# caiyuanhao1998/Open-DiffusionGS

Hardware: AMD Instinct MI355X
Metric: novel-view renders/sec (DiT step + GS raster) at 256^2 (higher is better)
Workload: dtype bf16; 1 GPU; obj-256 sampling step (BASELINE.json configs[2]): DGSDenoiser.forward = DiT image_to_gaussians (width 1024, 24 blocks, L=4098, bf16 MFMA, fp32 accumulate) + 4 fp32 rasterizations of P=262146 Gaussians at 256^2 per sample; random-init weights; batch_per_gpu=1, views=4, resolution=256, gaussians=262146, parallelism=dp1

## Files before the change

open-diffusiongs_amd/csrc/raster_forward.hip:

```cpp
#include <string.h>

#include "raster_cells.h"

namespace dgs {

struct FwdParams {
    int P, D, M, W, H, V, vps, gx, gy, T;
    const float *bg, *means3D, *shs, *colors_pre, *opac, *scales, *rots, *cov_pre, *viewm, *projm, *campos, *tanfov;
    float tanfovx, tanfovy, scale_mod;
    int prefiltered, raw_act;
    int bin_mode;
    int bitonic_cap;
    int bitonic_any;
    int exact_exp;
    int debug;
    int* radii;
    float* out_color;
    float *out_depth, *out_alpha;
    GeomState g;
    ImageState im;
    BinningState bn;
};

__device__ __forceinline__ void view_tanfov(const FwdParams& p, int v, float* tx, float* ty) {
    if (p.tanfov) { *tx = p.tanfov[2 * v]; *ty = p.tanfov[2 * v + 1]; }
    else { *tx = p.tanfovx; *ty = p.tanfovy; }
}

__device__ __forceinline__ void sh_to_rgb(int deg, const float* sh, float dx, float dy, float dz, float* out, unsigned* clamp_bits) {
    const float len = sqrtf(dx * dx + dy * dy + dz * dz);
    const float x = dx / len, y = dy / len, z = dz / len;
    unsigned bits = 0;
#pragma unroll
    for (int c = 0; c < 3; ++c) {
#define SH(k) sh[3 * (k) + c]
        float r = 0.28209479177387814f * SH(0);
        if (deg > 0) {
            r = r - 0.4886025119029199f * y * SH(1) + 0.4886025119029199f * z * SH(2) - 0.4886025119029199f * x * SH(3);
            if (deg > 1) {
                const float xx = x * x, yy = y * y, zz = z * z, xy = x * y, yz = y * z, xz = x * z;
                r = r + 1.0925484305920792f * xy * SH(4) + -1.0925484305920792f * yz * SH(5) +
                    0.31539156525252005f * (2.0f * zz - xx - yy) * SH(6) + -1.0925484305920792f * xz * SH(7) +
                    0.5462742152960396f * (xx - yy) * SH(8);
                if (deg > 2) {
                    r = r + -0.5900435899266435f * y * (3.0f * xx - yy) * SH(9) + 2.890611442640554f * xy * z * SH(10) +
                        -0.4570457994644658f * y * (4.0f * zz - xx - yy) * SH(11) +
                        0.3731763325901154f * z * (2.0f * zz - 3.0f * xx - 3.0f * yy) * SH(12) +
                        -0.4570457994644658f * x * (4.0f * zz - xx - yy) * SH(13) + 1.445305721320277f * z * (xx - yy) * SH(14) +
                        -0.5900435899266435f * x * (xx - 3.0f * yy) * SH(15);
                }
            }
        }
#undef SH
        r += 0.5f;
        if (r < 0) bits |= 1u << c;
        out[c] = fmaxf(r, 0.0f);
    }
    *clamp_bits = bits;
}

__device__ __forceinline__ bool preprocess_one(const FwdParams& p, int v, int idx, int* rx0, int* ry0, int* rx1, int* ry1, uint32_t* depth_key) {
    const int s = v / p.vps;
    const size_t gi = (size_t)v * p.P + idx;
    const size_t si = (size_t)s * p.P + idx;
    p.radii[gi] = 0;
    p.g.tiles_touched[gi] = 0;
    p.g.keys[0][gi] = 0xFFFFFFFFu;
    const float* vm = p.viewm + 16 * v;
    const float* pm = p.projm + 16 * v;
    const float mx = p.means3D[3 * si], my = p.means3D[3 * si + 1], mz = p.means3D[3 * si + 2];
    const float hx = pm[0] * mx + pm[4] * my + pm[8] * mz + pm[12];
    const float hy = pm[1] * mx + pm[5] * my + pm[9] * mz + pm[13];
    const float hw = pm[3] * mx + pm[7] * my + pm[11] * mz + pm[15];
    const float pw = 1.0f / (hw + 0.0000001f);
    const float projx = hx * pw, projy = hy * pw;
    float tx = vm[0] * mx + vm[4] * my + vm[8] * mz + vm[12];
    float ty = vm[1] * mx + vm[5] * my + vm[9] * mz + vm[13];
    const float tz = vm[2] * mx + vm[6] * my + vm[10] * mz + vm[14];
    if (tz <= 0.2f) {
        if (p.prefiltered) p.im.totals[1] = DGS_ERR_PREFILTERED_CULLED;
        return false;
    }
    float tanx, tany;
    view_tanfov(p, v, &tanx, &tany);
    const float focal_y = p.H / (2.0f * tany), focal_x = p.W / (2.0f * tanx);

    float c6[6];
    if (p.cov_pre) {
#pragma unroll
        for (int k = 0; k < 6; ++k) c6[k] = p.cov_pre[6 * si + k];
    } else {
        cov3d_from_scale_rot(p.scales + 3 * si, p.rots + 4 * si, p.raw_act != 0, p.scale_mod, c6);
        if (p.debug) {
#pragma unroll
            for (int k = 0; k < 6; ++k) p.g.cov3D[6 * gi + k] = c6[k];
        }
    }
    const float limx = 1.3f * tanx, limy = 1.3f * tany;
    const float txtz = tx / tz, tytz = ty / tz;
    tx = fminf(limx, fmaxf(-limx, txtz)) * tz;
    ty = fminf(limy, fmaxf(-limy, tytz)) * tz;
    const M3 J = m3_cols(focal_x / tz, 0.0f, -(focal_x * tx) / (tz * tz), 0.0f, focal_y / tz, -(focal_y * ty) / (tz * tz), 0, 0, 0);
    const M3 Wm = m3_cols(vm[0], vm[4], vm[8], vm[1], vm[5], vm[9], vm[2], vm[6], vm[10]);
    const M3 Tm = m3_mul(Wm, J);
    const M3 Vrk = m3_cols(c6[0], c6[1], c6[2], c6[1], c6[3], c6[4], c6[2], c6[4], c6[5]);
    const M3 cov = m3_mul(m3_mul(m3_t(Tm), m3_t(Vrk)), Tm);
    const float ca = cov.c[0][0] + 0.3f, cb = cov.c[0][1], cc = cov.c[1][1] + 0.3f;
    const float det = ca * cc - cb * cb;
    if (det == 0.0f) return false;
    const float det_inv = 1.f / det;
    const float conx = cc * det_inv, cony = -cb * det_inv, conz = ca * det_inv;
    const float mid = 0.5f * (ca + cc);
    const float l1 = mid + sqrtf(fmaxf(0.1f, mid * mid - det));
    const float l2 = mid - sqrtf(fmaxf(0.1f, mid * mid - det));
    const float my_radius = ceilf(3.f * sqrtf(fmaxf(l1, l2)));
    const float px = (float)(((projx + 1.0) * p.W - 1.0) * 0.5);
    const float py = (float)(((projy + 1.0) * p.H - 1.0) * 0.5);
    const int irad = f2i_sat(my_radius);
    int x0, y0, x1, y1;
    tile_rect(px, py, irad, p.gx, p.gy, &x0, &y0, &x1, &y1);
    if ((x1 - x0) * (y1 - y0) == 0) return false;
    float rgb[3];
    unsigned cbits = 0;
    if (p.colors_pre) {
        rgb[0] = p.colors_pre[3 * si]; rgb[1] = p.colors_pre[3 * si + 1]; rgb[2] = p.colors_pre[3 * si + 2];
    } else {
        const float* cam = p.campos + 3 * v;
        sh_to_rgb(p.D, p.shs + 3 * (size_t)p.M * si, mx - cam[0], my - cam[1], mz - cam[2], rgb, &cbits);
    }
    float op = p.opac[si];
    if (p.raw_act) op = 1.0f / (1.0f + det_expf(-op));
    const float cut = (op > 0.0f) ? (__logf(1.0f / (255.0f * op)) - 0.004f) : __builtin_inff();
    p.g.depths[gi] = tz;
    p.radii[gi] = irad;
    p.g.means2D[gi] = make_float2(px, py);
    BlendRecord* rec = p.g.blend + gi;
    rec->co = make_float4(conx, cony, conz, op);
    rec->rc = make_float4(rgb[0], rgb[1], rgb[2], cut);
    *reinterpret_cast<float4*>(&rec->xy) = make_float4(px, py, tz, 0.f);
    p.g.clamped[gi] = (uint8_t)cbits;
    p.g.tiles_touched[gi] = (uint32_t)((y1 - y0) * (x1 - x0));
    p.g.keys[0][gi] = __float_as_uint(tz);
    *depth_key = __float_as_uint(tz);
    *rx0 = x0; *ry0 = y0; *rx1 = x1; *ry1 = y1;
    return true;
}

template <bool LDS_HIST>
__global__ __launch_bounds__(256) void preprocess_kernel(FwdParams p) {
    DGS_DYNAMIC_LDS(smem);
    uint32_t* lhist = reinterpret_cast<uint32_t*>(smem);
    const int v = blockIdx.y;
    const int idx = blockIdx.x * 256 + threadIdx.x;
    if (LDS_HIST) {
        for (int i = threadIdx.x; i < p.T; i += 256) lhist[i] = 0;
        __syncthreads();
    }
    if (blockIdx.x == 0) {
        uint32_t* w = p.g.range_ws + (size_t)v * range_ws_stride(p.P);
        for (int i = threadIdx.x; i <= kRangeBuckets; i += 256) w[i] = 0u;
    }
    int x0 = 0, y0 = 0, x1 = 0, y1 = 0;
    bool vis = false;
    uint32_t depth_key = 0xFFFFFFFFu;
    if (idx < p.P) vis = preprocess_one(p, v, idx, &x0, &y0, &x1, &y1, &depth_key);
    {
        __shared__ uint32_t s_rng[2][4];
        const uint32_t key = vis ? depth_key : 0xFFFFFFFFu;
        uint32_t hi = key != 0xFFFFFFFFu ? key : 0u, lo_c = key != 0xFFFFFFFFu ? ~key : 0u;
#pragma unroll
        for (int o = 32; o > 0; o >>= 1) { hi = max(hi, (uint32_t)__shfl_xor((int)hi, o)); lo_c = max(lo_c, (uint32_t)__shfl_xor((int)lo_c, o)); }
        if ((threadIdx.x & 63) == 0) { s_rng[0][threadIdx.x >> 6] = hi; s_rng[1][threadIdx.x >> 6] = lo_c; }
        __syncthreads();
        if (threadIdx.x < 2) {
            const uint32_t m = max(max(s_rng[threadIdx.x][0], s_rng[threadIdx.x][1]), max(s_rng[threadIdx.x][2], s_rng[threadIdx.x][3]));
            if (m) atomicMax(p.im.depth_range + ((size_t)threadIdx.x * p.V + v) * kRangeSlots + (blockIdx.x % kRangeSlots), m);
        }
    }
    uint32_t* gcount = p.im.tile_count + (size_t)v * p.T;
    if (vis) {
        uint32_t* const grid = LDS_HIST ? lhist : gcount;
        atomicAdd(&grid[y0 * p.gx + x0], 1u);
        if (x1 < p.gx) atomicAdd(&grid[y0 * p.gx + x1], 0xffffffffu);
        if (y1 < p.gy) {
            atomicAdd(&grid[y1 * p.gx + x0], 0xffffffffu);
            if (x1 < p.gx) atomicAdd(&grid[y1 * p.gx + x1], 1u);
        }
    }
    if (LDS_HIST) {
        __syncthreads();
        for (int i = threadIdx.x; i < p.T; i += 256) {
            const uint32_t c = lhist[i];
            if (c) atomicAdd(&gcount[i], c);
        }
    }
}

__global__ __launch_bounds__(256) void radix_hist_kernel(const uint32_t* keys, uint32_t* hist, int P, int NB, int shift) {
    __shared__ uint32_t h[256];
    const int v = blockIdx.y, b = blockIdx.x;
    h[threadIdx.x] = 0;
    __syncthreads();
    const uint32_t* k = keys + (size_t)v * P;
    const int base = b * kSortTile;
#pragma unroll 4
    for (int r = 0; r < kSortItems; ++r) {
        const int i = base + r * 256 + threadIdx.x;
        if (i < P) atomicAdd(&h[(k[i] >> shift) & 255u], 1u);
    }
    __syncthreads();
    hist[((size_t)v * NB + b) * 256 + threadIdx.x] = h[threadIdx.x];
}

__global__ __launch_bounds__(256) void radix_colscan_kernel(uint32_t* hist, uint32_t* base, int NB) {
    __shared__ uint32_t scratch[8];
    const int v = blockIdx.y, d = threadIdx.x;
    uint32_t* h = hist + (size_t)v * NB * 256;
    uint32_t run = 0;
    for (int b0 = 0; b0 < NB; b0 += 16) {
        uint32_t c[16];
#pragma unroll
        for (int u = 0; u < 16; ++u) c[u] = (b0 + u < NB) ? h[(size_t)(b0 + u) * 256 + d] : 0u;
#pragma unroll
        for (int u = 0; u < 16; ++u) {
            if (b0 + u < NB) h[(size_t)(b0 + u) * 256 + d] = run;
            run += c[u];
        }
    }
    uint32_t total;
    const uint32_t ex = block_exclusive_scan<256>(run, scratch, &total);
    base[v * 256 + d] = ex;
}

__global__ __launch_bounds__(256) void radix_scatter_kernel(const uint32_t* keys_in, const uint32_t* vals_in, uint32_t* keys_out,
                                                           uint32_t* vals_out, uint32_t* rank_of, const uint32_t* hist,
                                                           const uint32_t* base, int P, int NB, int shift) {
    __shared__ uint32_t wcount[4][256];
    __shared__ uint32_t running[256];
    const int v = blockIdx.y, b = blockIdx.x, tid = threadIdx.x;
    const int lane = tid & 63, wave = tid >> 6;
    const size_t vo = (size_t)v * P;
    running[tid] = base[v * 256 + tid] + hist[((size_t)v * NB + b) * 256 + tid];
    const unsigned long long lt_mask = (lane == 0) ? 0ull : (~0ull >> (64 - lane));
    for (int r = 0; r < kSortItems; ++r) {
#pragma unroll
        for (int w = 0; w < 4; ++w) wcount[w][tid] = 0;
        __syncthreads();
        const int i = b * kSortTile + r * 256 + tid;
        const bool valid = i < P;
        const uint32_t key = valid ? keys_in[vo + i] : 0xFFFFFFFFu;
        const uint32_t val = valid ? (vals_in ? vals_in[vo + i] : (uint32_t)i) : 0u;
        const uint32_t dig = (key >> shift) & 255u;
        unsigned long long peers = __ballot(valid);
#pragma unroll
        for (int bit = 0; bit < 8; ++bit) {
            const unsigned long long m = __ballot((dig >> bit) & 1u);
            peers &= ((dig >> bit) & 1u) ? m : ~m;
        }
        const uint32_t rank_in_wave = (uint32_t)__popcll(peers & lt_mask);
        if (valid && rank_in_wave == 0) wcount[wave][dig] = (uint32_t)__popcll(peers);
        __syncthreads();
        if (valid) {
            uint32_t pos = running[dig] + rank_in_wave;
            for (int w = 0; w < wave; ++w) pos += wcount[w][dig];
            keys_out[vo + pos] = key;
            vals_out[vo + pos] = val;
            if (rank_of) rank_of[vo + val] = pos;
        }
        __syncthreads();
        running[tid] += wcount[0][tid] + wcount[1][tid] + wcount[2][tid] + wcount[3][tid];
    }
}

struct RangeMap {
    uint32_t lo; float scale; bool any;
    __device__ __forceinline__ uint32_t bucket(uint32_t key) const { return min((uint32_t)((float)(key - lo) * scale), (uint32_t)kRangeBuckets - 1u); }
};
__device__ __forceinline__ RangeMap range_map(const uint32_t* depth_range, int V, int v, uint32_t* s_map ) {
    if (threadIdx.x < 64) {
        const int which = threadIdx.x >> 5, slot = threadIdx.x & 31;
        uint32_t x = slot < kRangeSlots ? depth_range[((size_t)which * V + v) * kRangeSlots + slot] : 0u;
#pragma unroll
        for (int o = 16; o > 0; o >>= 1) x = max(x, (uint32_t)__shfl_xor((int)x, o));
        if (slot == 0) s_map[which] = x;
    }
    __syncthreads();
    const uint32_t hi_w = s_map[0], lo_w = s_map[1];
    const uint32_t hi = hi_w, lo = ~lo_w;
    RangeMap m;
    m.any = (hi_w | lo_w) != 0u;
    m.lo = m.any ? lo : 0u;
    m.scale = m.any ? (float)kRangeBuckets / ((float)(hi - lo) + 1.0f) : 0.f;
    return m;
}

__global__ __launch_bounds__(256) void range_count_kernel(const uint32_t* keys, const uint32_t* depth_range, uint32_t* ws, int P, int V, int stride) {
    __shared__ uint32_t h[kRangeBuckets];
    __shared__ uint32_t s_c[4];
    __shared__ uint32_t s_map[2];
    const int v = blockIdx.y, b = blockIdx.x, tid = threadIdx.x;
    const RangeMap m = range_map(depth_range, V, v, s_map);
    for (int i = tid; i < kRangeBuckets; i += 256) h[i] = 0;
    __syncthreads();
    const uint32_t* k = keys + (size_t)v * P;
    uint32_t culled = 0;
#pragma unroll 4
    for (int r = 0; r < kRangeItems; ++r) {
        const int i = b * kRangeTile + r * 256 + tid;
        if (i < P) {
            const uint32_t key = k[i];
            if (key != 0xFFFFFFFFu) atomicAdd(&h[m.bucket(key)], 1u); else ++culled;
        }
    }
#pragma unroll
    for (int o = 32; o > 0; o >>= 1) culled += (uint32_t)__shfl_xor((int)culled, o);
    if ((tid & 63) == 0) s_c[tid >> 6] = culled;
    __syncthreads();
    uint32_t* w = ws + (size_t)v * stride;
    for (int i = tid; i < kRangeBuckets; i += 256) { const uint32_t c = h[i]; if (c) atomicAdd(&w[i], c); }
    if (tid == 0) w[2 * kRangeBuckets + 1 + b] = (s_c[0] + s_c[1]) + (s_c[2] + s_c[3]);
}

__global__ __launch_bounds__(1024) void range_plan_kernel(uint32_t* ws, int NB, int NWIN, int stride) {
    __shared__ uint32_t scratch[20];
    __shared__ uint32_t s_start[kRangeBuckets + 1];
    uint32_t* w = ws + (size_t)blockIdx.x * stride;
    const int tid = threadIdx.x;
    const uint32_t c = tid < kRangeBuckets ? w[tid] : 0u;
    uint32_t nvis;
    const uint32_t ex = block_exclusive_scan<1024>(c, scratch, &nvis);
    __syncthreads();
    if (tid < kRangeBuckets) { w[tid] = ex; w[kRangeBuckets + 1 + tid] = 0u; s_start[tid] = ex; }
    if (tid == 0) { w[kRangeBuckets] = nvis; s_start[kRangeBuckets] = nvis; }
    __syncthreads();
    for (int j = tid; j <= NWIN; j += 1024) {
        const uint32_t want = (uint32_t)j * (uint32_t)kRangeWindow;
        int lo = 0, hi = kRangeBuckets;
        while (lo < hi) { const int mid = (lo + hi) >> 1; if (s_start[mid] < want) lo = mid + 1; else hi = mid; }
        w[2 * kRangeBuckets + 1 + NB + j] = j == NWIN ? nvis : s_start[lo];
    }
    const uint32_t cc = tid < NB ? w[2 * kRangeBuckets + 1 + tid] : 0u;
    uint32_t all;
    const uint32_t cex = block_exclusive_scan<1024>(cc, scratch, &all);
    if (tid < NB) w[2 * kRangeBuckets + 1 + tid] = nvis + cex;
}

__global__ __launch_bounds__(256) void range_scatter_kernel(const uint32_t* keys, const uint32_t* depth_range, uint32_t* ws, uint32_t* keys_out,
                                                           uint32_t* vals_out, uint32_t* order, uint32_t* rank_of, int P, int V, int stride) {
    __shared__ uint32_t h[kRangeBuckets];
    __shared__ uint32_t s_cc[kRangeItems][4];
    __shared__ uint32_t s_map[2];
    const int v = blockIdx.y, b = blockIdx.x, tid = threadIdx.x, lane = tid & 63, wave = tid >> 6;
    const RangeMap m = range_map(depth_range, V, v, s_map);
    const size_t vo = (size_t)v * P;
    uint32_t* w = ws + (size_t)v * stride;
    for (int i = tid; i < kRangeBuckets; i += 256) h[i] = 0;
    __syncthreads();
    uint32_t key[kRangeItems], slot[kRangeItems];
    const unsigned long long lt_mask = (lane == 0) ? 0ull : (~0ull >> (64 - lane));
#pragma unroll
    for (int r = 0; r < kRangeItems; ++r) {
        const int i = b * kRangeTile + r * 256 + tid;
        key[r] = i < P ? keys[vo + i] : 0u;
        const bool in = i < P, cul = in && key[r] == 0xFFFFFFFFu;
        slot[r] = (in && !cul) ? atomicAdd(&h[m.bucket(key[r])], 1u) : 0u;
        const unsigned long long cm = __ballot(cul);
        if (cul) slot[r] = (uint32_t)__popcll(cm & lt_mask);
        if (lane == 0) s_cc[r][wave] = (uint32_t)__popcll(cm);
    }
    __syncthreads();
    {
        constexpr int Q = kRangeBuckets / 256;
        uint32_t c[Q], st0[Q], got[Q];
#pragma unroll
        for (int q = 0; q < Q; ++q) { c[q] = h[tid + 256 * q]; st0[q] = w[tid + 256 * q]; }
#pragma unroll
        for (int q = 0; q < Q; ++q) got[q] = c[q] ? atomicAdd(&w[kRangeBuckets + 1 + tid + 256 * q], c[q]) : 0u;
#pragma unroll
        for (int q = 0; q < Q; ++q) h[tid + 256 * q] = st0[q] + got[q];
    }
    __syncthreads();
    const uint32_t cbase = w[2 * kRangeBuckets + 1 + b];
#pragma unroll
    for (int r = 0; r < kRangeItems; ++r) {
        const int i = b * kRangeTile + r * 256 + tid;
        if (i >= P) continue;
        if (key[r] != 0xFFFFFFFFu) {
            const uint32_t pos = h[m.bucket(key[r])] + slot[r];
            keys_out[vo + pos] = key[r];
            vals_out[vo + pos] = (uint32_t)i;
        } else {
            uint32_t off = 0;
            for (int q = 0; q < r; ++q) off += (s_cc[q][0] + s_cc[q][1]) + (s_cc[q][2] + s_cc[q][3]);
            for (int q = 0; q < wave; ++q) off += s_cc[r][q];
            const uint32_t pos = cbase + off + slot[r];
            order[vo + pos] = (uint32_t)i;
            rank_of[vo + i] = pos;
        }
    }
}

__global__ __launch_bounds__(1024) void scan_tiles_kernel(uint32_t* count, uint2* ranges, uint32_t* cursor, int n,
                                                         int32_t* totals, long long capacity, uint32_t* order, int gx, int gy,
                                                         int32_t* stats_dev, int32_t* stats_host) {
    __shared__ uint32_t scratch[20];
    __shared__ uint32_t smax;
    __shared__ uint32_t s_class[1024];
    {
        const int T = gx * gy, V = n / T;
        for (int r = threadIdx.x; r < V * gy; r += 1024) {
            uint32_t* row = count + (size_t)(r / gy) * T + (size_t)(r % gy) * gx;
            uint32_t run = 0;
            for (int x0 = 0; x0 < gx; x0 += 16) {
                uint32_t c[16];
#pragma unroll
                for (int u = 0; u < 16; ++u) c[u] = x0 + u < gx ? row[x0 + u] : 0u;
#pragma unroll
                for (int u = 0; u < 16; ++u)
                    if (x0 + u < gx) { run += c[u]; row[x0 + u] = run; }
            }
        }
        __syncthreads();
        for (int cidx = threadIdx.x; cidx < V * gx; cidx += 1024) {
            uint32_t* col = count + (size_t)(cidx / gx) * T + (cidx % gx);
            uint32_t run = 0;
            for (int y0 = 0; y0 < gy; y0 += 16) {
                uint32_t c[16];
#pragma unroll
                for (int u = 0; u < 16; ++u) c[u] = y0 + u < gy ? col[(size_t)(y0 + u) * gx] : 0u;
#pragma unroll
                for (int u = 0; u < 16; ++u)
                    if (y0 + u < gy) { run += c[u]; col[(size_t)(y0 + u) * gx] = run; }
            }
        }
        __syncthreads();
    }
    uint32_t carry = 0, mx = 0;
    if (threadIdx.x == 0) smax = 0;
    for (int base = 0; base < n; base += 1024) {
        const int i = base + threadIdx.x;
        const uint32_t c = (i < n) ? count[i] : 0u;
        mx = max(mx, c);
        uint32_t tot;
        const uint32_t ex = block_exclusive_scan<1024>(c, scratch, &tot);
        if (i < n) { ranges[i] = make_uint2(carry + ex, carry + ex + c); cursor[i] = 0; }
        carry += tot;
    }
    __syncthreads();
    atomicMax(&smax, mx);
    __syncthreads();
    if (threadIdx.x == 0) {
        totals[0] = (int32_t)carry;
        totals[2] = (int32_t)smax;
        if (capacity >= 0 && (long long)carry > capacity) totals[1] = DGS_ERR_BINNING_OVERFLOW;
        const int32_t st1 = totals[1];
        if (stats_dev) { stats_dev[0] = (int32_t)carry; stats_dev[1] = st1; stats_dev[2] = (int32_t)smax; stats_dev[3] = 1; }
        if (stats_host) {
            stats_host[0] = (int32_t)carry; stats_host[1] = st1; stats_host[2] = (int32_t)smax;
            __threadfence_system();
            *reinterpret_cast<volatile int32_t*>(stats_host + 3) = 1;
        }
    }
    deal_tiles(count, n, smax, order, s_class, scratch);
}

enum { kFormRankSort = 1, kFormScan = 2, kFormBitonic = 3 };
__host__ __device__ __forceinline__ int binning_form_of(int bin_mode, int bitonic_cap, long long num_rendered, long long longest,
                                                        long long T, long long P, long long V, bool any_len = false) {
    const bool fits = bitonic_cap > 0 && (any_len || longest <= bitonic_cap);
    if (bin_mode == kFormScan || bin_mode == kFormRankSort) return bin_mode;
    if (bin_mode == kFormBitonic) return fits ? kFormBitonic : kFormRankSort;
    if (num_rendered * 10 >= T * P * V) return kFormScan;
    return fits ? kFormBitonic : kFormRankSort;
}
__host__ __device__ __forceinline__ bool scan_form_possible(int gx, int gy, long long T, long long P) {
    return gx <= 255 && gy <= 255 && T * P <= (1ll << 31);
}
__device__ __forceinline__ int binning_form(const FwdParams& p) {
    return binning_form_of(p.bin_mode, p.bitonic_cap, (long long)(uint32_t)p.im.totals[0], (long long)(uint32_t)p.im.totals[2], p.T, p.P, p.V,
                           p.bitonic_any != 0);
}
__device__ __forceinline__ bool binning_is_scan(const FwdParams& p) { return binning_form(p) == kFormScan; }

template <bool LDS_AGG>
__global__ __launch_bounds__(256) void emit_instances_kernel(FwdParams p) {
    DGS_DYNAMIC_LDS(smem);
    uint32_t* lcnt = reinterpret_cast<uint32_t*>(smem);
    uint32_t* lbase = lcnt + p.T;
    const int form = binning_form(p);
    if (p.im.totals[1] != 0 || form == kFormScan) return;
    const bool wide = form == kFormBitonic;
    const int v = blockIdx.y;
    const int idx = blockIdx.x * 256 + threadIdx.x;
    const size_t gi = (size_t)v * p.P + idx;
    int x0 = 0, y0 = 0, x1 = 0, y1 = 0;
    bool vis = false;
    if (idx < p.P && p.radii[gi] > 0) {
// ... 423 lines not shown
            const unsigned long long m = __ballot(tx - x0 < x1 - x0) & __ballot(ty - y0 < y1 - y0);
            if (EMIT) {
                const bool set = (m >> lane) & 1ull;
                slot[u] = off + cnt + (uint32_t)__popcll(m & lanes_before);
                val[u] = set ? order[rank0 + 64u * u] : 0u;
                setm |= (uint32_t)set << u;
            }
            cnt += (uint32_t)__popcll(m);
        }
        if (EMIT) {
#pragma unroll
            for (int u = 0; u < 8; ++u)
                if (((setm >> u) & 1u) && list_at + slot[u] < list_cap) {
                    ring[(ring_at + slot[u]) & (kRing - 1u)] = val[u];
                    list[list_at + slot[u]] = val[u];
                }
        }
    }
    return cnt;
}

__device__ __forceinline__ void scan_more(const FwdParams& p, TileScan& s, uint32_t* ring, uint32_t* scratch, const uint32_t* rects,
                                          const uint32_t* order, uint32_t* list, uint32_t count, uint32_t tx, uint32_t ty, int lane, int wave,
                                          unsigned long long lanes_before) {
    const uint32_t P = (uint32_t)p.P;
    unsigned long long want = 768ull * P / (count ? count : 1u);
    uint32_t win = (uint32_t)(want > (1ull << 24) ? (1ull << 24) : want);
    win = max(1024u, (win + 255u) & ~255u);
    const uint32_t room = kRing - s.waiting;
    uint32_t total = 0, off = 0;
    int g0 = 0, g1 = 0;
    for (;;) {
        const int groups = (int)((min(win, P - s.next_rank) + 63u) / 64u);
        const int gpw = (groups + 3) / 4;
        g0 = wave * gpw; g1 = min(groups, g0 + gpw);
        const uint32_t cnt = scan_groups<false>(rects, order, s.next_rank, g0, g1, P, tx, ty, lane, lanes_before, 0u, nullptr, 0u, nullptr, 0u, 0u);
        if (lane == 0) scratch[wave] = cnt;
        __syncthreads();
        total = 0; off = 0;
#pragma unroll
        for (int w = 0; w < 4; ++w) {
            const uint32_t c = scratch[w];
            if (w < wave) off += c;
            total += c;
        }
        __syncthreads();
        if (total <= room || win <= 256u) break;
        win = max(256u, (win / 2u + 255u) & ~255u);
    }
    scan_groups<true>(rects, order, s.next_rank, g0, g1, P, tx, ty, lane, lanes_before, off, ring, s.head + s.waiting, list, s.found, count);
    __syncthreads();
    s.next_rank += min(win, P - s.next_rank);
    s.found += total;
    s.waiting += total;
}

template <bool SCAN, bool FAST_EXP, bool AUX = false>
__global__ __launch_bounds__(256) void blend_forward_kernel(FwdParams p) {
    __shared__ CellXY<AUX> s_xy[256];
    __shared__ float4 s_co[256];
    __shared__ float4 s_rgbc[256];
    __shared__ uint4 s_cnt[16];
    __shared__ uint8_t s_list[17][256];
    __shared__ uint32_t s_walk[4];
    __shared__ uint2 s_stat[kRasterStats ? 4 : 1];
    __shared__ uint32_t s_ring[SCAN ? kRing : 1];
    __shared__ uint32_t s_scan[4];
    if (binning_is_scan(p) != SCAN) return;
    const uint32_t vt = p.im.tile_order[blockIdx.x];
    const int v = (int)(vt / (uint32_t)p.T), tile = (int)(vt % (uint32_t)p.T);
    const int bx = tile % p.gx, by = tile / p.gx;
    const int tid = threadIdx.x, lane = tid & 63, row = lane >> 4;
    const int wave = __builtin_amdgcn_readfirstlane(tid >> 6);
    const int cell = wave * 4 + row;
    const int pxi = bx * kTile + 4 * row + (lane & 3), pyi = by * kTile + 4 * wave + ((lane >> 2) & 3);
    const bool inside = pxi < p.W && pyi < p.H;
    const float pfx = (float)pxi, pfy = (float)pyi;
    const float tx0 = (float)(bx * kTile), ty0 = (float)(by * kTile);
    const unsigned long long lanes_before = (lane == 0) ? 0ull : (~0ull >> (64 - lane));
    const bool ok = p.im.totals[1] == 0;
    uint2 rg = p.im.ranges[vt];
    if (!ok) rg.y = rg.x;
    const int rounds = (int)((rg.y - rg.x + 255u) / 256u);
    const size_t vo = (size_t)v * p.P;
    const uint32_t* rects = p.g.vals[1] + vo;
    const uint32_t* order = p.g.vals[0] + vo;
    TileScan ts{0u, 0u, 0u, 0u};
    bool done = !inside;
    float T = 1.0f, C0 = 0.f, C1 = 0.f, C2 = 0.f;
    float Dz = 0.f;
    uint32_t last_contributor = 0;
    uint32_t st_entries = 0, st_trips = 0, st_batches = 0;
    for (int i = 0; i < rounds; ++i) {
        if (__syncthreads_count(done) == 256) break;
        if constexpr (kRasterStats) ++st_batches;
        const uint32_t pos = rg.x + (uint32_t)i * 256u + (uint32_t)tid;
        const uint32_t need = min(256u, rg.y - rg.x - (uint32_t)i * 256u);
        if (SCAN) {
            while (ts.waiting < need && ts.next_rank < (uint32_t)p.P)
                scan_more(p, ts, s_ring, s_scan, rects, order, p.bn.point_list + rg.x, rg.y - rg.x, (uint32_t)bx, (uint32_t)by, lane, wave, lanes_before);
        }
        const bool has = pos < rg.y && (!SCAN || (uint32_t)tid < ts.waiting);
        uint32_t id = 0u;
        if (has) id = SCAN ? s_ring[(ts.head + (uint32_t)tid) & (kRing - 1u)] : p.bn.point_list[pos];
        const unsigned m16[1] = {stage_entry<AUX>(has, p.g.blend + vo, nullptr, id, tid, tx0, ty0, s_xy, s_co, s_rgbc)};
        const uint32_t kept = compact_cells<1>(m16, cell, tid, lane, wave, lanes_before, s_cnt, s_list);
        if (SCAN) { const uint32_t took = min(need, ts.waiting); ts.head += took; ts.waiting -= took; }
        const uint32_t base = (uint32_t)i * 256u;
        const unsigned long long alive = __ballot(!done);
        if (alive != 0ull) {
            const uint32_t tot = (((alive >> (16 * row)) & 0xFFFFull) != 0ull) ? kept : 0u;
            uint32_t tot_l = done ? 0u : tot;
            using Entry = CellEntry<AUX>;
            auto load = [&](uint32_t j) { return Entry{s_xy[j], s_co[j], s_rgbc[j]}; };
            auto step = [&](uint32_t k, uint32_t j, const Entry& e) {
                const float dx = e.xy.x - pfx, dy = e.xy.y - pfy;
                const float power = -0.5f * (e.co.x * dx * dx + e.co.z * dy * dy) - e.co.y * dx * dy;
                const bool pass = (k < tot_l) & !(power > 0.0f) & !(power < e.rc.w);
                if (wave_ballot(pass) != 0ull) {
                    const float alpha = alpha_clamp(e.co.w * blend_exp<FAST_EXP>(pass ? power : 0.0f, e.co.w));
                    const float test_T = T * (1 - alpha);
                    const bool contributes = pass & !(alpha < 1.0f / 255.0f);
                    const bool finishes = contributes & (test_T < 0.0001f);
                    const bool blends = contributes & !finishes;
                    tot_l = finishes ? 0u : tot_l;
                    if constexpr (FAST_EXP) {
                        const float w = blends ? alpha * T : 0.0f;
                        C0 = __builtin_fmaf(e.rc.x, w, C0); C1 = __builtin_fmaf(e.rc.y, w, C1); C2 = __builtin_fmaf(e.rc.z, w, C2);
                        if constexpr (AUX) Dz = __builtin_fmaf(e.xy.z, w, Dz);
                    } else {
                        const float c0 = C0 + e.rc.x * alpha * T, c1 = C1 + e.rc.y * alpha * T, c2 = C2 + e.rc.z * alpha * T;
                        C0 = blends ? c0 : C0;
                        C1 = blends ? c1 : C1;
                        C2 = blends ? c2 : C2;
                        if constexpr (AUX) { const float dz = Dz + e.xy.z * alpha * T; Dz = blends ? dz : Dz; }
                    }
                    T = blends ? test_T : T;
                    last_contributor = blends ? base + j + 1u : last_contributor;
                }
            };
            const uint32_t k = walk_cell(s_list[cell], load, step, [&](uint32_t at) { return wave_ballot(at < tot_l) != 0ull; });
            done = done | (tot_l != tot);
            if constexpr (kRasterStats) { st_entries += min(tot, k); st_trips += k; }
        }
    }
    if (inside) {
        const size_t pid = (size_t)p.W * pyi + pxi;
        const size_t HW = (size_t)p.H * p.W;
        p.im.final_T[(size_t)v * HW + pid] = T;
        p.im.n_contrib[(size_t)v * HW + pid] = last_contributor;
        float* out = p.out_color + (size_t)v * 3 * HW;
        const float bad = __uint_as_float(0x7FC00000u);
        out[pid] = ok ? C0 + T * p.bg[0] : bad;
        out[HW + pid] = ok ? C1 + T * p.bg[1] : bad;
        out[2 * HW + pid] = ok ? C2 + T * p.bg[2] : bad;
        if constexpr (AUX) {
            p.out_depth[(size_t)v * HW + pid] = ok ? Dz : bad;
            p.out_alpha[(size_t)v * HW + pid] = ok ? 1.0f - T : bad;
        }
    }
    uint32_t walked = last_contributor;
#pragma unroll
    for (int o = 32; o > 0; o >>= 1) walked = max(walked, (uint32_t)__shfl_xor((int)walked, o));
    uint2 stat = make_uint2(0u, 0u);
    if constexpr (kRasterStats) stat = tile_stat_sums<4>((lane & 15) == 0, st_entries, st_trips, lane, wave, s_stat);
    if (lane == 0) s_walk[wave] = walked;
    __syncthreads();
    if (tid == 0) {
        p.im.tile_work[vt] = max(max(s_walk[0], s_walk[1]), max(s_walk[2], s_walk[3]));
        p.im.tile_cursor[vt] = SCAN ? ts.found : rg.y - rg.x;
        p.im.tile_scanned[vt] = SCAN ? ts.next_rank : 0u;
        if constexpr (kRasterStats) p.im.tile_stats[vt] = make_uint4(stat.x, stat.y, SCAN ? ts.next_rank : 0u, st_batches);
    }
}

__global__ __launch_bounds__(1024) void zero_words_kernel(uint32_t* dst, int n) {
    for (int i = threadIdx.x; i < n; i += 1024) dst[i] = 0u;
}

__global__ void record_field_kernel(const BlendRecord* rec, float4* dst, size_t n, int field) {
    const size_t i = (size_t)blockIdx.x * 256 + threadIdx.x;
    if (i < n) dst[i] = field ? rec[i].rc : rec[i].co;
}

__global__ void mark_visible_kernel(int P, const float* means, const float* vm, uint8_t* present) {
    const int i = blockIdx.x * 256 + threadIdx.x;
    if (i >= P) return;
    const float mx = means[3 * i], my = means[3 * i + 1], mz = means[3 * i + 2];
    const float tz = vm[2] * mx + vm[6] * my + vm[10] * mz + vm[14];
    present[i] = !(tz <= 0.2f);
}

template <bool SCAN>
static void launch_blend_forward(const FwdParams& p, bool aux, int VT, size_t lds_pad, hipStream_t st) {
    with_flag(!p.exact_exp, [&](auto fast) {
        with_flag(aux, [&](auto ax) {
            hipLaunchKernelGGL((blend_forward_kernel<SCAN, decltype(fast)::value, decltype(ax)::value>), dim3(VT), dim3(256), lds_pad, st, p);
        });
    });
}

static int check(hipStream_t st, int debug) {
    hipError_t e = debug ? hipStreamSynchronize(st) : hipSuccess;
    if (e == hipSuccess) e = hipGetLastError();
    if (e != hipSuccess) { fprintf(stderr, "[dgs] rasterizer: HIP error %d (%s)\n", (int)e, hipGetErrorString(e)); return DGS_ERR_DEVICE; }
    return DGS_OK;
}

static int pick_window_words(int P) {
    int words = (P + 31) / 32;
    words = ((words + 255) / 256) * 256;
    const int kMax = 16128;
    return words < kMax ? words : kMax;
}

}

using namespace dgs;

extern "C" {

int dgs_abi_version(void) { return DGS_ABI_VERSION; }

const char* dgs_status_string(int s) {
    switch (s) {
        case DGS_OK: return "ok";
        case DGS_ERR_INVALID_ARGUMENT: return "invalid argument (means3D must have dimensions (num_points, 3); sizes must be positive)";
        case DGS_ERR_NEED_COLORS: return "provide exactly one of SHs or precomputed colors";
        case DGS_ERR_NEED_COVARIANCE: return "provide exactly one of scale/rotation pair or precomputed 3D covariance";
        case DGS_ERR_ALLOC: return "state-buffer allocation failed";
        case DGS_ERR_DEVICE: return "HIP device error";
        case DGS_ERR_PREFILTERED_CULLED: return "point is filtered although prefiltered is set";
        case DGS_ERR_BINNING_OVERFLOW: return "num_rendered exceeds binning capacity";
        default: return "unknown status";
    }
}

size_t dgs_raster_geom_bytes(int32_t P, int32_t V) { size_t b; GeomState::carve(nullptr, (size_t)P, (size_t)V, &b); return b; }
size_t dgs_raster_image_bytes(int32_t W, int32_t H, int32_t V) { size_t b; ImageState::carve(nullptr, (size_t)W, (size_t)H, (size_t)V, &b); return b; }
size_t dgs_raster_binning_bytes(int64_t N) { size_t b; BinningState::carve(nullptr, (size_t)(N < 1 ? 1 : N), &b); return b; }

int dgs_raster_forward(DgsRasterForwardArgs* a, dgs_stream_t stream) {
    hipStream_t st = static_cast<hipStream_t>(stream);
    if (!a || a->P < 0 || a->width <= 0 || a->height <= 0 || a->V < 1 || a->views_per_set < 1) return DGS_ERR_INVALID_ARGUMENT;
    const int P = a->P, V = a->V, W = a->width, H = a->height;
    a->num_rendered = 0;
    (void)hipGetLastError();
    if (!a->out_color || !a->geom_alloc || !a->img_alloc || !a->binning_alloc) return DGS_ERR_INVALID_ARGUMENT;
    if ((a->out_depth == nullptr) != (a->out_alpha == nullptr)) return DGS_ERR_INVALID_ARGUMENT;
    const bool aux = a->out_depth != nullptr;
    const size_t HW = (size_t)W * H;
    if (P == 0) {
        hipMemsetAsync(a->out_color, 0, (size_t)V * 3 * HW * sizeof(float), st);
        if (aux) { hipMemsetAsync(a->out_depth, 0, (size_t)V * HW * sizeof(float), st); hipMemsetAsync(a->out_alpha, 0, (size_t)V * HW * sizeof(float), st); }
        return check(st, a->debug);
    }
    if (!a->means3D || !a->opacities || !a->viewmatrix || !a->projmatrix || !a->campos || !a->background || !a->radii) return DGS_ERR_INVALID_ARGUMENT;
    if ((a->shs == nullptr) == (a->colors_precomp == nullptr)) return DGS_ERR_NEED_COLORS;
    if (a->cov3D_precomp ? (a->scales || a->rotations) : !(a->scales && a->rotations)) return DGS_ERR_NEED_COVARIANCE;
    if (a->shs && (a->M < 1 || a->D < 0 || (a->D + 1) * (a->D + 1) > a->M || a->D > 3)) return DGS_ERR_INVALID_ARGUMENT;

    FwdParams p{};
    p.P = P; p.D = a->D; p.M = a->M; p.W = W; p.H = H; p.V = V; p.vps = a->views_per_set;
    p.gx = (W + kTile - 1) / kTile; p.gy = (H + kTile - 1) / kTile; p.T = p.gx * p.gy;
    p.bg = a->background; p.means3D = a->means3D; p.shs = a->shs; p.colors_pre = a->colors_precomp; p.opac = a->opacities;
    p.scales = a->scales; p.rots = a->rotations; p.cov_pre = a->cov3D_precomp; p.viewm = a->viewmatrix; p.projm = a->projmatrix;
    p.campos = a->campos; p.tanfov = a->tanfov; p.tanfovx = a->tanfovx; p.tanfovy = a->tanfovy; p.scale_mod = a->scale_modifier;
    p.prefiltered = a->prefiltered; p.raw_act = a->raw_activations; p.radii = a->radii; p.out_color = a->out_color;
    p.out_depth = a->out_depth; p.out_alpha = a->out_alpha;
    p.exact_exp = a->exact_exp ? 1 : 0;
    p.debug = a->debug ? 1 : 0;

    size_t gbytes, ibytes;
    GeomState::carve(nullptr, (size_t)P, (size_t)V, &gbytes);
    ImageState::carve(nullptr, (size_t)W, (size_t)H, (size_t)V, &ibytes);
    void* gbuf = a->geom_alloc(gbytes, a->geom_user);
    void* ibuf = a->img_alloc(ibytes, a->img_user);
    if (!gbuf || !ibuf) return DGS_ERR_ALLOC;
    p.g = GeomState::carve(gbuf, (size_t)P, (size_t)V, nullptr);
    p.im = ImageState::carve(ibuf, (size_t)W, (size_t)H, (size_t)V, nullptr);
    const bool async = a->binning_capacity > 0;
    void* bbuf = nullptr;
    if (async) {
        bbuf = a->binning_alloc(dgs_raster_binning_bytes(a->binning_capacity), a->binning_user);
        if (!bbuf) return DGS_ERR_ALLOC;
        p.bn = BinningState::carve(bbuf, (size_t)a->binning_capacity, nullptr);
    }

    const int VT = V * p.T;
    constexpr int kBitonicMax = 16384;
    static const bool lds_ok =
        hipFuncSetAttribute(reinterpret_cast<const void*>(tile_bitonic_kernel<256>), hipFuncAttributeMaxDynamicSharedMemorySize,
                            kBitonicMax * 8 + 2 * kBuckets * 4) == hipSuccess &&
        hipFuncSetAttribute(reinterpret_cast<const void*>(tile_bitonic_kernel<1024>), hipFuncAttributeMaxDynamicSharedMemorySize,
                            kBitonicMax * 8 + 2 * kBuckets * 4) == hipSuccess &&
        hipFuncSetAttribute(reinterpret_cast<const void*>(tile_bitonic_kernel<512>), hipFuncAttributeMaxDynamicSharedMemorySize,
                            kBitonicMax * 8 + 2 * kBuckets * 4) == hipSuccess &&
        hipFuncSetAttribute(reinterpret_cast<const void*>(range_sort_kernel<512>), hipFuncAttributeMaxDynamicSharedMemorySize,
                            kRangeSortCap * 8 + 2 * kBuckets * 4) == hipSuccess;
    if (!lds_ok) { fprintf(stderr, "[dgs] rasterizer: hipFuncSetAttribute(tile_bitonic_kernel, %d bytes of LDS) failed\n", kBitonicMax * 8 + 2 * kBuckets * 4); return DGS_ERR_DEVICE; }
    hipLaunchKernelGGL(zero_words_kernel, dim3(1), dim3(1024), 0, st, p.im.tile_count, (int)p.im.zero_span((size_t)V));
    const dim3 gridP((P + 255) / 256, V);
    const bool lds_tiles = p.T <= 4096;
    if (lds_tiles) hipLaunchKernelGGL((preprocess_kernel<true>), gridP, dim3(256), (size_t)p.T * 4, st, p);
    else hipLaunchKernelGGL((preprocess_kernel<false>), gridP, dim3(256), 0, st, p);
    int rc = check(st, a->debug);
    if (rc) return rc;

    const bool can_scan = scan_form_possible(p.gx, p.gy, p.T, P);
    p.bin_mode = a->binning_form;
    if (p.bin_mode < 0 || p.bin_mode > 3 || (p.bin_mode == 0 && !can_scan) || (p.bin_mode == kFormScan && !can_scan)) p.bin_mode = can_scan ? 0 : kFormBitonic;
    int bitonic_only_cap = 0;
    if (async && p.bin_mode == kFormBitonic && a->longest_hint > 0) {
        bitonic_only_cap = 2048;
        while (bitonic_only_cap < a->longest_hint + a->longest_hint / 2 && bitonic_only_cap < kBitonicMax) bitonic_only_cap <<= 1;
    }
    hipLaunchKernelGGL(scan_tiles_kernel, dim3(1), dim3(1024), 0, st, p.im.tile_count, p.im.ranges, p.im.tile_cursor, VT, p.im.totals,
                       async ? (long long)a->binning_capacity : -1LL, p.im.tile_order, p.gx, p.gy, a->num_rendered_dev, a->num_rendered_host);
    rc = check(st, a->debug);
    if (rc) return rc;

    int forms = 0;
    static thread_local int last_form = 0;
    bool radix_done = false;
    auto radix_sort = [&]() {
        const int NB = sort_blocks(P);
        static const bool use_radix = getenv("DGS_RASTER_SORT") && !strcmp(getenv("DGS_RASTER_SORT"), "radix");
        const int RB = range_blocks(P);
        if (!use_radix && RB <= 1024) {
            const int stride = (int)range_ws_stride(P);
            hipLaunchKernelGGL(range_count_kernel, dim3(RB, V), dim3(256), 0, st, p.g.keys[0], p.im.depth_range, p.g.range_ws, P, V, stride);
            const int NWIN = range_windows(P), seg_off = 2 * kRangeBuckets + 1 + RB;
            hipLaunchKernelGGL(range_plan_kernel, dim3(V), dim3(1024), 0, st, p.g.range_ws, RB, NWIN, stride);
            hipLaunchKernelGGL(range_scatter_kernel, dim3(RB, V), dim3(256), 0, st, p.g.keys[0], p.im.depth_range, p.g.range_ws, p.g.keys[1], p.g.vals[1],
                               p.g.vals[0], p.g.rank_of, P, V, stride);
            hipLaunchKernelGGL(range_sort_kernel<512>, dim3(NWIN, V), dim3(512), kRangeSortCap * 8 + 2 * kBuckets * 4, st, p.g.range_ws, p.g.keys[1], p.g.vals[1],
                               p.g.vals[0], p.g.rank_of, P, stride, seg_off);
            radix_done = true;
            return;
        }
        for (int pass = 0; pass < 4; ++pass) {
            const int in = pass & 1, out = in ^ 1;
            hipLaunchKernelGGL(radix_hist_kernel, dim3(NB, V), dim3(256), 0, st, p.g.keys[in], p.g.radix_hist, P, NB, 8 * pass);
            hipLaunchKernelGGL(radix_colscan_kernel, dim3(1, V), dim3(256), 0, st, p.g.radix_hist, p.g.radix_base, NB);
            hipLaunchKernelGGL(radix_scatter_kernel, dim3(NB, V), dim3(256), 0, st, p.g.keys[in], pass == 0 ? (const uint32_t*)nullptr : p.g.vals[in],
                               p.g.keys[out], p.g.vals[out], pass == 3 ? p.g.rank_of : (uint32_t*)nullptr, p.g.radix_hist, p.g.radix_base, P, NB, 8 * pass);
        }
        radix_done = true;
    };
    if (!async) {
        if (last_form != kFormBitonic && p.bin_mode != kFormBitonic) radix_sort();
        int32_t tot[4] = {0, 0, 0, 0};
        if (hipMemcpyAsync(tot, p.im.totals, sizeof(tot), hipMemcpyDeviceToHost, st) != hipSuccess) return DGS_ERR_DEVICE;
        if (hipStreamSynchronize(st) != hipSuccess) return DGS_ERR_DEVICE;
        if (tot[1] != 0) return tot[1];
        a->num_rendered = (int64_t)(uint32_t)tot[0];
        a->longest_list = (int64_t)(uint32_t)tot[2];
        bbuf = a->binning_alloc(dgs_raster_binning_bytes(a->num_rendered), a->binning_user);
        if (!bbuf) return DGS_ERR_ALLOC;
        p.bn = BinningState::carve(bbuf, (size_t)(a->num_rendered < 1 ? 1 : a->num_rendered), nullptr);
        int cap = 2048;
        while (cap < tot[2] && cap < kBitonicMax) cap <<= 1;
        p.bitonic_cap = cap;
        last_form = binning_form_of(p.bin_mode, p.bitonic_cap, a->num_rendered, (uint32_t)tot[2], p.T, P, V);
        forms = 1 << last_form;
    } else {
        a->num_rendered = -1;
        a->longest_list = -1;
        p.bitonic_cap = bitonic_only_cap ? bitonic_only_cap : kBitonicMax;
        p.bitonic_any = bitonic_only_cap ? 1 : 0;
        forms = p.bin_mode ? (1 << p.bin_mode) | (p.bin_mode == kFormBitonic && !bitonic_only_cap ? 1 << kFormRankSort : 0)
                           : (1 << kFormRankSort) | (1 << kFormScan) | (1 << kFormBitonic);
    }

    size_t blend_pad = 0;
    if constexpr (kRasterAblate) { static const int pad = [] { const char* e = getenv("DGS_RASTER_FWD_LDS_PAD"); return e ? atoi(e) : 0; }(); blend_pad = (size_t)pad; }
    if ((forms & ((1 << kFormRankSort) | (1 << kFormScan))) && !radix_done) radix_sort();
    if (forms & (1 << kFormScan)) {
        hipLaunchKernelGGL(rank_rects_kernel, gridP, dim3(256), 0, st, p);
        launch_blend_forward<true>(p, aux, VT, blend_pad, st);
    }
    if (forms & ((1 << kFormRankSort) | (1 << kFormBitonic))) {
        if (lds_tiles) hipLaunchKernelGGL((emit_instances_kernel<true>), gridP, dim3(256), (size_t)p.T * 8, st, p);
        else hipLaunchKernelGGL((emit_instances_kernel<false>), gridP, dim3(256), 0, st, p);
    }
    if (forms & (1 << kFormRankSort)) {
        const int wwords = pick_window_words(P);
        hipLaunchKernelGGL(tile_sort_kernel, dim3(p.T, V), dim3(256), (size_t)wwords * 4, st, p, wwords);
    }
    if (forms & (1 << kFormBitonic)) {
        const size_t lds = (size_t)p.bitonic_cap * 8 + 2 * kBuckets * 4;
        static const int nt_env = getenv("DGS_RASTER_BITONIC_NT") ? atoi(getenv("DGS_RASTER_BITONIC_NT")) : 0;
        if (p.bitonic_cap > 8192) hipLaunchKernelGGL(tile_bitonic_kernel<1024>, dim3(VT), dim3(1024), lds, st, p);
        else if (p.bitonic_cap >= 4096 && nt_env != 256) hipLaunchKernelGGL(tile_bitonic_kernel<512>, dim3(VT), dim3(512), lds, st, p);
        else hipLaunchKernelGGL(tile_bitonic_kernel<256>, dim3(VT), dim3(256), lds, st, p);
    }
    if (forms & ((1 << kFormRankSort) | (1 << kFormBitonic))) launch_blend_forward<false>(p, aux, VT, blend_pad, st);
    return check(st, a->debug);
}

int dgs_raster_binning_form(int32_t binning_form, int64_t num_rendered, int64_t longest_list, int32_t P, int32_t W, int32_t H, int32_t V) {
    if (P < 0 || W <= 0 || H <= 0 || V < 1 || num_rendered < 0 || longest_list < 0) return DGS_ERR_INVALID_ARGUMENT;
    const int gx = (W + kTile - 1) / kTile, gy = (H + kTile - 1) / kTile;
    const long long T = (long long)gx * gy;
    const bool can_scan = scan_form_possible(gx, gy, T, P);
    int mode = binning_form;
    if (mode < 0 || mode > 3 || (mode == 0 && !can_scan) || (mode == kFormScan && !can_scan)) mode = can_scan ? 0 : kFormBitonic;
    return binning_form_of(mode, 16384, num_rendered, longest_list, T, P, V);
}

int dgs_mark_visible(int32_t P, const float* means3D, const float* viewmatrix, const float* projmatrix, uint8_t* present,
                     dgs_stream_t stream) {
    (void)projmatrix;
    if (P < 0) return DGS_ERR_INVALID_ARGUMENT;
    if (P == 0) return DGS_OK;
    if (!means3D || !viewmatrix || !present) return DGS_ERR_INVALID_ARGUMENT;
    hipStream_t st = static_cast<hipStream_t>(stream);
    hipLaunchKernelGGL(mark_visible_kernel, dim3((P + 255) / 256), dim3(256), 0, st, P, means3D, viewmatrix, present);
    return hipGetLastError() == hipSuccess ? DGS_OK : DGS_ERR_DEVICE;
}

int64_t dgs_raster_state_read(const char* name, int32_t P, int32_t W, int32_t H, int32_t V, int64_t N, const void* gbuf,
                              const void* bbuf, const void* ibuf, void* dst, int64_t dst_bytes, dgs_stream_t stream) {
    hipStream_t st = static_cast<hipStream_t>(stream);
    const GeomState g = GeomState::carve(const_cast<void*>(gbuf), (size_t)P, (size_t)V, nullptr);
    const ImageState im = ImageState::carve(const_cast<void*>(ibuf), (size_t)W, (size_t)H, (size_t)V, nullptr);
    const BinningState bn = BinningState::carve(const_cast<void*>(bbuf), (size_t)(N < 1 ? 1 : N), nullptr);
    const size_t n = (size_t)P * V, HW = (size_t)W * H * V;
    const size_t T = (size_t)((W + kTile - 1) / kTile) * ((H + kTile - 1) / kTile) * V;
    const void* src = nullptr;
    size_t bytes = 0;
    const auto is = [&](const char* s) { return strcmp(name, s) == 0; };
    if (is("depths")) { src = g.depths; bytes = n * 4; }
    else if (is("means2D")) { src = g.means2D; bytes = n * 8; }
    else if (is("conic_opacity") || is("rgb")) {
        bytes = n * 16;
        if ((int64_t)bytes > dst_bytes) return DGS_ERR_INVALID_ARGUMENT;
        if (n) hipLaunchKernelGGL(record_field_kernel, dim3((unsigned)((n + 255) / 256)), dim3(256), 0, st, g.blend, static_cast<float4*>(dst), n, is("rgb") ? 1 : 0);
        return hipGetLastError() == hipSuccess ? (int64_t)bytes : (int64_t)DGS_ERR_DEVICE;
    }
    else if (is("tiles_touched")) { src = g.tiles_touched; bytes = n * 4; }
    else if (is("clamped")) { src = g.clamped; bytes = n; }
    else if (is("cov3D")) { src = g.cov3D; bytes = n * 24; }
    else if (is("rank_of")) { src = g.rank_of; bytes = n * 4; }
    else if (is("order")) { src = g.vals[0]; bytes = n * 4; }
    else if (is("ranges")) { src = im.ranges; bytes = T * 8; }
    else if (is("n_contrib")) { src = im.n_contrib; bytes = HW * 4; }
    else if (is("final_T")) { src = im.final_T; bytes = HW * 4; }
    else if (is("list_len")) { src = im.tile_cursor; bytes = T * 4; }
    else if (is("tile_work")) { src = im.tile_work; bytes = T * 4; }
    else if (is("tile_scanned")) { src = im.tile_scanned; bytes = T * 4; }
    else if (is("tile_stats")) { src = im.tile_stats; bytes = T * 16; }
    else if (is("tile_stats_bwd")) { src = im.tile_stats + T; bytes = T * 16; }
    else if (is("point_list")) { src = bn.point_list; bytes = (size_t)(N < 0 ? 0 : N) * 4; }
    else return DGS_ERR_INVALID_ARGUMENT;
    if ((int64_t)bytes > dst_bytes) return DGS_ERR_INVALID_ARGUMENT;
    if (bytes && hipMemcpyAsync(dst, src, bytes, hipMemcpyDeviceToDevice, st) != hipSuccess) return DGS_ERR_DEVICE;
    return (int64_t)bytes;
}

}
```

Measured before the change: 685.0 renders/s.

## Preprocess all views of a sample in one kernel, loading each Gaussian once

Adds a preprocess_set_kernel in which each thread loads a Gaussian's inputs (mean, 3D covariance, opacity, view-independent colour) once and then projects it for every view of the same sample. The per-view LDS tile histograms and depth-range reductions are kept in shared memory for all views. This removes the repeated global loads and the repeated covariance and sigmoid work across the 4 views. It also defers the invisible-path stores so they are written only on cull. In exchange, the kernel uses more LDS per block and launches fewer blocks. A debug field-export hook for keys, tile_count and tile_order is also added.

New measurement: 686.8 renders/s, median of 6. No clear change (+0.3%).

```diff
diff --git a/open-diffusiongs_amd/csrc/raster_forward.hip b/open-diffusiongs_amd/csrc/raster_forward.hip
--- a/open-diffusiongs_amd/csrc/raster_forward.hip
+++ b/open-diffusiongs_amd/csrc/raster_forward.hip
@@ -59,16 +59,43 @@
     *clamp_bits = bits;
 }
 
-__device__ __forceinline__ bool preprocess_one(const FwdParams& p, int v, int idx, int* rx0, int* ry0, int* rx1, int* ry1, uint32_t* depth_key) {
-    const int s = v / p.vps;
+struct GaussInputs {
+    float mx, my, mz;
+    float c6[6];
+    float op, cut;
+    float rgb[3];
+    unsigned cbits;
+};
+__device__ __forceinline__ bool view_free_colour(const FwdParams& p) { return p.colors_pre != nullptr || p.D == 0; }
+
+__device__ __forceinline__ void preprocess_load(const FwdParams& p, int s, int idx, GaussInputs* g) {
+    const size_t si = (size_t)s * p.P + idx;
+    g->mx = p.means3D[3 * si]; g->my = p.means3D[3 * si + 1]; g->mz = p.means3D[3 * si + 2];
+    if (p.cov_pre) {
+#pragma unroll
+        for (int k = 0; k < 6; ++k) g->c6[k] = p.cov_pre[6 * si + k];
+    } else {
+        cov3d_from_scale_rot(p.scales + 3 * si, p.rots + 4 * si, p.raw_act != 0, p.scale_mod, g->c6);
+    }
+    g->cbits = 0;
+    g->rgb[0] = g->rgb[1] = g->rgb[2] = 0.f;
+    if (p.colors_pre) {
+        g->rgb[0] = p.colors_pre[3 * si]; g->rgb[1] = p.colors_pre[3 * si + 1]; g->rgb[2] = p.colors_pre[3 * si + 2];
+    } else if (p.D == 0) {
+        sh_to_rgb(0, p.shs + 3 * (size_t)p.M * si, 1.f, 0.f, 0.f, g->rgb, &g->cbits);
+    }
+    float op = p.opac[si];
+    if (p.raw_act) op = 1.0f / (1.0f + det_expf(-op));
+    g->op = op;
+    g->cut = (op > 0.0f) ? (__logf(1.0f / (255.0f * op)) - 0.004f) : __builtin_inff();
+}
+
+__device__ __forceinline__ bool preprocess_visible(const FwdParams& p, int v, int idx, const GaussInputs& g, int* rx0, int* ry0, int* rx1, int* ry1,
+                                                uint32_t* depth_key) {
     const size_t gi = (size_t)v * p.P + idx;
-    const size_t si = (size_t)s * p.P + idx;
-    p.radii[gi] = 0;
-    p.g.tiles_touched[gi] = 0;
-    p.g.keys[0][gi] = 0xFFFFFFFFu;
     const float* vm = p.viewm + 16 * v;
     const float* pm = p.projm + 16 * v;
-    const float mx = p.means3D[3 * si], my = p.means3D[3 * si + 1], mz = p.means3D[3 * si + 2];
+    const float mx = g.mx, my = g.my, mz = g.mz;
     const float hx = pm[0] * mx + pm[4] * my + pm[8] * mz + pm[12];
     const float hy = pm[1] * mx + pm[5] * my + pm[9] * mz + pm[13];
     const float hw = pm[3] * mx + pm[7] * my + pm[11] * mz + pm[15];
@@ -85,16 +112,10 @@
     view_tanfov(p, v, &tanx, &tany);
     const float focal_y = p.H / (2.0f * tany), focal_x = p.W / (2.0f * tanx);
 
-    float c6[6];
-    if (p.cov_pre) {
-#pragma unroll
-        for (int k = 0; k < 6; ++k) c6[k] = p.cov_pre[6 * si + k];
-    } else {
-        cov3d_from_scale_rot(p.scales + 3 * si, p.rots + 4 * si, p.raw_act != 0, p.scale_mod, c6);
-        if (p.debug) {
-#pragma unroll
-            for (int k = 0; k < 6; ++k) p.g.cov3D[6 * gi + k] = c6[k];
-        }
+    const float* c6 = g.c6;
+    if (!p.cov_pre && p.debug) {
+#pragma unroll
+        for (int k = 0; k < 6; ++k) p.g.cov3D[6 * gi + k] = c6[k];
     }
     const float limx = 1.3f * tanx, limy = 1.3f * tany;
     const float txtz = tx / tz, tytz = ty / tz;
@@ -120,23 +141,18 @@
     int x0, y0, x1, y1;
     tile_rect(px, py, irad, p.gx, p.gy, &x0, &y0, &x1, &y1);
     if ((x1 - x0) * (y1 - y0) == 0) return false;
-    float rgb[3];
-    unsigned cbits = 0;
-    if (p.colors_pre) {
-        rgb[0] = p.colors_pre[3 * si]; rgb[1] = p.colors_pre[3 * si + 1]; rgb[2] = p.colors_pre[3 * si + 2];
-    } else {
+    float rgb[3] = {g.rgb[0], g.rgb[1], g.rgb[2]};
+    unsigned cbits = g.cbits;
+    if (!view_free_colour(p)) {
         const float* cam = p.campos + 3 * v;
-        sh_to_rgb(p.D, p.shs + 3 * (size_t)p.M * si, mx - cam[0], my - cam[1], mz - cam[2], rgb, &cbits);
-    }
-    float op = p.opac[si];
-    if (p.raw_act) op = 1.0f / (1.0f + det_expf(-op));
-    const float cut = (op > 0.0f) ? (__logf(1.0f / (255.0f * op)) - 0.004f) : __builtin_inff();
+        sh_to_rgb(p.D, p.shs + 3 * (size_t)p.M * ((size_t)(v / p.vps) * p.P + idx), mx - cam[0], my - cam[1], mz - cam[2], rgb, &cbits);
+    }
     p.g.depths[gi] = tz;
     p.radii[gi] = irad;
     p.g.means2D[gi] = make_float2(px, py);
     BlendRecord* rec = p.g.blend + gi;
-    rec->co = make_float4(conx, cony, conz, op);
-    rec->rc = make_float4(rgb[0], rgb[1], rgb[2], cut);
+    rec->co = make_float4(conx, cony, conz, g.op);
+    rec->rc = make_float4(rgb[0], rgb[1], rgb[2], g.cut);
     *reinterpret_cast<float4*>(&rec->xy) = make_float4(px, py, tz, 0.f);
     p.g.clamped[gi] = (uint8_t)cbits;
     p.g.tiles_touched[gi] = (uint32_t)((y1 - y0) * (x1 - x0));
@@ -144,6 +160,24 @@
     *depth_key = __float_as_uint(tz);
     *rx0 = x0; *ry0 = y0; *rx1 = x1; *ry1 = y1;
     return true;
+}
+__device__ __forceinline__ bool preprocess_view(const FwdParams& p, int v, int idx, const GaussInputs& g, int* rx0, int* ry0, int* rx1, int* ry1,
+                                                uint32_t* depth_key) {
+    if (preprocess_visible(p, v, idx, g, rx0, ry0, rx1, ry1, depth_key)) return true;
+    const size_t gi = (size_t)v * p.P + idx;
+    p.radii[gi] = 0;
+    p.g.tiles_touched[gi] = 0;
+    p.g.keys[0][gi] = 0xFFFFFFFFu;
+    return false;
+}
+
+__device__ __forceinline__ void add_rect_corners(uint32_t* grid, int gx, int gy, int x0, int y0, int x1, int y1) {
+    atomicAdd(&grid[y0 * gx + x0], 1u);
+    if (x1 < gx) atomicAdd(&grid[y0 * gx + x1], 0xffffffffu);
+    if (y1 < gy) {
+        atomicAdd(&grid[y1 * gx + x0], 0xffffffffu);
+        if (x1 < gx) atomicAdd(&grid[y1 * gx + x1], 1u);
+    }
 }
 
 template <bool LDS_HIST>
@@ -163,7 +197,11 @@
     int x0 = 0, y0 = 0, x1 = 0, y1 = 0;
     bool vis = false;
     uint32_t depth_key = 0xFFFFFFFFu;
-    if (idx < p.P) vis = preprocess_one(p, v, idx, &x0, &y0, &x1, &y1, &depth_key);
+    if (idx < p.P) {
+        GaussInputs g;
+        preprocess_load(p, v / p.vps, idx, &g);
+        vis = preprocess_view(p, v, idx, g, &x0, &y0, &x1, &y1, &depth_key);
+    }
     {
         __shared__ uint32_t s_rng[2][4];
         const uint32_t key = vis ? depth_key : 0xFFFFFFFFu;
@@ -178,21 +216,54 @@
         }
     }
     uint32_t* gcount = p.im.tile_count + (size_t)v * p.T;
-    if (vis) {
-        uint32_t* const grid = LDS_HIST ? lhist : gcount;
-        atomicAdd(&grid[y0 * p.gx + x0], 1u);
-        if (x1 < p.gx) atomicAdd(&grid[y0 * p.gx + x1], 0xffffffffu);
-        if (y1 < p.gy) {
-            atomicAdd(&grid[y1 * p.gx + x0], 0xffffffffu);
-            if (x1 < p.gx) atomicAdd(&grid[y1 * p.gx + x1], 1u);
-        }
-    }
+    if (vis) add_rect_corners(LDS_HIST ? lhist : gcount, p.gx, p.gy, x0, y0, x1, y1);
     if (LDS_HIST) {
         __syncthreads();
         for (int i = threadIdx.x; i < p.T; i += 256) {
             const uint32_t c = lhist[i];
             if (c) atomicAdd(&gcount[i], c);
         }
+    }
+}
+
+__global__ __launch_bounds__(256) void preprocess_set_kernel(FwdParams p, int vpt) {
+    DGS_DYNAMIC_LDS(smem);
+    uint32_t* lhist = reinterpret_cast<uint32_t*>(smem);
+    uint32_t* s_rng = lhist + (size_t)vpt * p.T;
+    const int v0 = blockIdx.y * vpt;
+    const int idx = blockIdx.x * 256 + threadIdx.x;
+    for (int i = threadIdx.x; i < vpt * p.T; i += 256) lhist[i] = 0;
+    __syncthreads();
+    if (blockIdx.x == 0) {
+        for (int j = 0; j < vpt; ++j) {
+            uint32_t* w = p.g.range_ws + (size_t)(v0 + j) * range_ws_stride(p.P);
+            for (int i = threadIdx.x; i <= kRangeBuckets; i += 256) w[i] = 0u;
+        }
+    }
+    GaussInputs g;
+    if (idx < p.P) preprocess_load(p, v0 / p.vps, idx, &g);
+    for (int j = 0; j < vpt; ++j) {
+        int x0 = 0, y0 = 0, x1 = 0, y1 = 0;
+        uint32_t depth_key = 0xFFFFFFFFu;
+        const bool vis = idx < p.P && preprocess_view(p, v0 + j, idx, g, &x0, &y0, &x1, &y1, &depth_key);
+        const uint32_t key = vis ? depth_key : 0xFFFFFFFFu;
+        uint32_t hi = key != 0xFFFFFFFFu ? key : 0u, lo_c = key != 0xFFFFFFFFu ? ~key : 0u;
+#pragma unroll
+        for (int o = 32; o > 0; o >>= 1) { hi = max(hi, (uint32_t)__shfl_xor((int)hi, o)); lo_c = max(lo_c, (uint32_t)__shfl_xor((int)lo_c, o)); }
+        if ((threadIdx.x & 63) == 0) { s_rng[8 * j + (threadIdx.x >> 6)] = hi; s_rng[8 * j + 4 + (threadIdx.x >> 6)] = lo_c; }
+        if (vis) add_rect_corners(lhist + (size_t)j * p.T, p.gx, p.gy, x0, y0, x1, y1);
+    }
+    __syncthreads();
+    if (threadIdx.x < 2 * vpt) {
+        const int j = threadIdx.x >> 1, which = threadIdx.x & 1;
+        const uint32_t* r = s_rng + 8 * j + 4 * which;
+        const uint32_t m = max(max(r[0], r[1]), max(r[2], r[3]));
+        if (m) atomicMax(p.im.depth_range + ((size_t)which * p.V + (v0 + j)) * kRangeSlots + (blockIdx.x % kRangeSlots), m);
+    }
+    uint32_t* gcount = p.im.tile_count + (size_t)v0 * p.T;
+    for (int i = threadIdx.x; i < vpt * p.T; i += 256) {
+        const uint32_t c = lhist[i];
+        if (c) atomicAdd(&gcount[i], c);
     }
 }
 
@@ -1222,7 +1293,11 @@
     hipLaunchKernelGGL(zero_words_kernel, dim3(1), dim3(1024), 0, st, p.im.tile_count, (int)p.im.zero_span((size_t)V));
     const dim3 gridP((P + 255) / 256, V);
     const bool lds_tiles = p.T <= 4096;
-    if (lds_tiles) hipLaunchKernelGGL((preprocess_kernel<true>), gridP, dim3(256), (size_t)p.T * 4, st, p);
+    static const int pre_env = [] { const char* e = getenv("DGS_RASTER_PREPROCESS"); return !e ? 0 : !strcmp(e, "per_view") ? 1 : atoi(e); }();
+    int vpt = pre_env > 0 ? pre_env : p.vps;
+    if (vpt < 1 || p.vps % vpt != 0 || V % p.vps != 0 || !lds_tiles || (size_t)vpt * ((size_t)p.T * 4 + 32) > 32768) vpt = 1;
+    if (vpt > 1) hipLaunchKernelGGL(preprocess_set_kernel, dim3((P + 255) / 256, V / vpt), dim3(256), (size_t)vpt * ((size_t)p.T * 4 + 32), st, p, vpt);
+    else if (lds_tiles) hipLaunchKernelGGL((preprocess_kernel<true>), gridP, dim3(256), (size_t)p.T * 4, st, p);
     else hipLaunchKernelGGL((preprocess_kernel<false>), gridP, dim3(256), 0, st, p);
     int rc = check(st, a->debug);
     if (rc) return rc;
@@ -1364,6 +1439,9 @@
     else if (is("cov3D")) { src = g.cov3D; bytes = n * 24; }
     else if (is("rank_of")) { src = g.rank_of; bytes = n * 4; }
     else if (is("order")) { src = g.vals[0]; bytes = n * 4; }
+    else if (is("keys")) { src = g.keys[0]; bytes = n * 4; }
+    else if (is("tile_count")) { src = im.tile_count; bytes = T * 4; }
+    else if (is("tile_order")) { src = im.tile_order; bytes = T * 4; }
     else if (is("ranges")) { src = im.ranges; bytes = T * 8; }
     else if (is("n_contrib")) { src = im.n_contrib; bytes = HW * 4; }
     else if (is("final_T")) { src = im.final_T; bytes = HW * 4; }
```
